# aleju/gan-reverser

Hardware: AMD Instinct MI355X
Metric: images/sec G+R fwd/bwd (higher is better)
Workload: dtype f32 via f16x3 (2-term fp16 split of power-of-two-scaled operands, 3 MFMA products, fp32 accumulate); 1 GPU; 32x32 grayscale, noise=32, batch=256/GPU: G fwd + R fwd/bwd + Adam; global_batch=256, per_gpu_batch=256, parallelism=dp1, bn=per-rank batch statistics

## Files before the change

gan-reverser_amd/csrc/elem.hip:

```cpp
#include "kernels.h"
#include "colorspace.h"
#include <type_traits>

namespace gr {

__device__ __forceinline__ double block_reduce_sum(double v, double* sh) {
#pragma unroll
  for (int off = 32; off > 0; off >>= 1) v += __shfl_down(v, off, 64);
  const int lane = threadIdx.x & 63, wave = threadIdx.x >> 6, nw = (blockDim.x + 63) >> 6;
  __syncthreads();
  if (lane == 0) sh[wave] = v;
  __syncthreads();
  double r = 0;
  if (threadIdx.x == 0) for (int w = 0; w < nw; ++w) r += sh[w];
  return r;
}

__device__ __forceinline__ unsigned udivp(unsigned x, unsigned d) { return (d & (d - 1)) == 0 ? x >> (__ffs(d) - 1) : x / d; }
__device__ __forceinline__ float post_slope(const PostArgs& a) { return a.act == ACT_PRELU ? *a.slope_dev : a.slope; }
template <int CB>
__device__ __forceinline__ void post_specialize(PostArgs& f) {
  if (CB == 1) { f.act = ACT_ELU; f.has_bn = 1; f.m1.kind = MASK_ELEM; f.pool = 0; f.m2.kind = MASK_NONE; }
  if (CB == 2) { f.act = ACT_ELU; f.has_bn = 1; f.m1.kind = MASK_NONE; f.pool = POOL_MAX; f.m2.kind = MASK_ELEM; }
  if (CB == 3) { f.act = ACT_ELU; f.has_bn = 1; f.m1.kind = MASK_SPATIAL; f.pool = POOL_MAX; f.m2.kind = MASK_NONE; }
// ... 1032 lines not shown
  PostBwdArgs a = a0;
  a.nt = 0;
  const PostArgs& f = a.f;
  const double pre = (double)f.B * f.C * f.H * f.W, post = f.pool ? pre / 4 : pre;
  const bool vec = (f.pool ? (f.W % 8 == 0 && f.H % 2 == 0) : (f.W % 4 == 0)) && f.H * f.W >= 64 && pre < 4.0e9;
  if (vec) {
    long blocks = ((long)(pre / 4) + 255) / 256;
    if (blocks > 8192) blocks = 8192;
    KtScope kt("post_backward_frozen_vec_kernel", 0.0, 4.0 * (2.0 * pre + post), s);
    with_combo(post_combo(f), [&](auto cb) { hipLaunchKernelGGL(post_backward_frozen_vec_kernel<decltype(cb)::value>, dim3((unsigned)blocks), dim3(256), 0, s, a); });
  } else {
    long blocks = ((long)pre + 255) / 256;
    if (blocks > 8192) blocks = 8192;
    if (blocks < 1) blocks = 1;
    KtScope kt("post_backward_frozen_kernel", 0.0, 4.0 * (2.0 * pre + post), s);
    hipLaunchKernelGGL(post_backward_frozen_kernel, dim3((unsigned)blocks), dim3(256), 0, s, a);
  }
}

__global__ __launch_bounds__(256) void channel_absmax_kernel(const float* __restrict__ t, int B, long HW, long sB, long sC, unsigned* __restrict__ chmax) {
  const int c = blockIdx.x;
  const long n = (long)B * HW;
  float m = 0.f;
  for (long j = (long)blockIdx.y * 256 + threadIdx.x; j < n; j += (long)gridDim.y * 256) {
    const long b = j / HW, i = j - b * HW;
    m = fmaxf(m, fabsf(t[b * sB + (long)c * sC + i]));
  }
#pragma unroll
  for (int off = 32; off > 0; off >>= 1) m = fmaxf(m, __shfl_down(m, off, 64));
  if ((threadIdx.x & 63) == 0 && m > 0.f) atomicMax(chmax + c, __float_as_uint(m));
}
__device__ __forceinline__ void spread_enter(float mx, float mn, unsigned* word, int side) {
  __shared__ float tmx[256], tmn[256];
  tmx[threadIdx.x] = mx; tmn[threadIdx.x] = mn;
  __syncthreads();
  if (threadIdx.x == 0) {
    for (int i = 1; i < 256; ++i) { mx = fmaxf(mx, tmx[i]); mn = fminf(mn, tmn[i]); }
    if (mx > 0.f && mn < mx) {
      const unsigned bits = (unsigned)min(ilogbf(mx) - ilogbf(mn) + 1, 0xffff);
      const unsigned w = *word;
      unsigned a = w & 0xffffu, b = w >> 16;
      if (side == 0) a = max(a, bits); else b = max(b, bits);
      *word = a | b << 16;
    }
  }
}
__global__ __launch_bounds__(256) void spread_verdict_kernel(unsigned* chmax, int C, unsigned* word, int side) {
  float mx = 0.f, mn = INFINITY;
  for (int c = threadIdx.x; c < C; c += 256) {
    const float v = __uint_as_float(chmax[c]); chmax[c] = 0u;
    mx = fmaxf(mx, v); if (v > 0.f) mn = fminf(mn, v);
  }
  spread_enter(mx, mn, word, side);
}
__global__ __launch_bounds__(256) void pair_spread_kernel(const float* __restrict__ a, const float* __restrict__ b, int C, unsigned* word) {
  float mx = 0.f, mn = INFINITY;
  for (int c = threadIdx.x; c < C; c += 256) {
    const float v = fmaxf(fabsf(a[c]), b ? fabsf(b[c]) : 0.f);
    mx = fmaxf(mx, v); if (v > 0.f) mn = fminf(mn, v);
  }
  spread_enter(mx, mn, word, 0);
}
void launch_channel_absmax(const float* t, int B, int C, long HW, long sB, long sC, unsigned* chmax, hipStream_t s) {
  const long n = (long)B * HW;
  int splits = (int)((n + 4095) / 4096);
  if (splits < 1) splits = 1;
  if ((long)splits * C > 8192) splits = (int)(8192 / C > 0 ? 8192 / C : 1);
  KtScope kt("range_guard_scan", 0.0, 4.0 * (double)n * C, s);
  hipLaunchKernelGGL(channel_absmax_kernel, dim3(C, splits), dim3(256), 0, s, t, B, HW, sB, sC, chmax);
}
void launch_spread_verdict(unsigned* chmax, int C, unsigned* word, int side, hipStream_t s) {
  hipLaunchKernelGGL(spread_verdict_kernel, dim3(1), dim3(256), 0, s, chmax, C, word, side);
}
void launch_pair_spread(const float* a, const float* b, int C, unsigned* sides, hipStream_t s) {
  hipLaunchKernelGGL(pair_spread_kernel, dim3(1), dim3(256), 0, s, a, b, C, sides);
}

__global__ __launch_bounds__(1024) void mse_kernel(const float* __restrict__ x, const float* __restrict__ t, long n, double inv_n,
                                                   float norm, double* loss, float* grad) {
  __shared__ double sh[16];
  double s = 0;
  for (long i = threadIdx.x; i < n; i += blockDim.x) {
    const float z = x[i] - t[i];
    s += (double)(z * z);
    if (grad) grad[i] = norm * z;
  }
  s = block_reduce_sum(s, sh);
  if (threadIdx.x == 0 && loss) *loss = s * inv_n;
}
void launch_mse(const float* x, const float* t, long n, long n_global, double* loss_dev, float* grad, hipStream_t s) {
  hipLaunchKernelGGL(mse_kernel, dim3(1), dim3(1024), 0, s, x, t, n, 1.0 / (double)n_global, (float)(2.0 / (double)n_global), loss_dev, grad);
}

__global__ __launch_bounds__(256) void mse_rows_kernel(const float* __restrict__ x, const float* __restrict__ t, long n, double inv_n, float norm,
                                                       float* __restrict__ loss_rows, float* __restrict__ grad) {
  __shared__ double sh[8];
  const long base = (long)blockIdx.x * n;
  double s = 0;
  for (long j = threadIdx.x; j < n; j += blockDim.x) {
    const float z = x[base + j] - t[base + j];
    s += (double)z * (double)z;
    if (grad) grad[base + j] = norm * z;
  }
  s = block_reduce_sum(s, sh);
  if (threadIdx.x == 0) loss_rows[blockIdx.x] = (float)(s * inv_n);
}
void launch_mse_rows(const float* x, const float* t, long rows, long n, float* loss_rows, float* grad, hipStream_t s) {
  KtScope kt("mse_rows_kernel", 3.0 * (double)rows * n, 4.0 * (double)rows * n * (grad ? 3.0 : 2.0), s);
  hipLaunchKernelGGL(mse_rows_kernel, dim3((unsigned)rows), dim3(256), 0, s, x, t, n, 1.0 / (double)n, (float)(2.0 / (double)n), loss_rows, grad);
}

#define HEAD_KEEP8(a_, i_) asm volatile("" :: "v"((a_)[(i_)]), "v"((a_)[(i_) + 1]), "v"((a_)[(i_) + 2]), "v"((a_)[(i_) + 3]), "v"((a_)[(i_) + 4]), "v"((a_)[(i_) + 5]), "v"((a_)[(i_) + 6]), "v"((a_)[(i_) + 7]))
#define HEAD_KEEP16(a_, i_) asm volatile("" :: "v"((a_)[(i_)]), "v"((a_)[(i_) + 1]), "v"((a_)[(i_) + 2]), "v"((a_)[(i_) + 3]), "v"((a_)[(i_) + 4]), "v"((a_)[(i_) + 5]), "v"((a_)[(i_) + 6]), "v"((a_)[(i_) + 7]), \
                                              "v"((a_)[(i_) + 8]), "v"((a_)[(i_) + 9]), "v"((a_)[(i_) + 10]), "v"((a_)[(i_) + 11]), "v"((a_)[(i_) + 12]), "v"((a_)[(i_) + 13]), "v"((a_)[(i_) + 14]), "v"((a_)[(i_) + 15]))
__device__ __forceinline__ unsigned head_mask_word(const MaskRef& m, long e) { return m.bits[e >> 5]; }
__device__ __forceinline__ float head_mask_of(const MaskRef& m, unsigned w, long e) { const float k = ((w >> (e & 31)) & 1u) ? m.scale : 0.f; return m.kind == MASK_ELEM ? k : 1.f; }
struct HeadArgs {
  int B, C1, nd, rows_per_wg;
  const float* y1; float* out1;
  float* mean; float* invstd; float* run_mean; float* run_var; const float* gamma; const float* beta;
  MaskRef m1; int act1; float slope1; int act2;
  const float* W2; const float* b2; float* y2; float* out2;
  const float* target; double inv_n; float norm; double* loss; double* loss_part;
  float* gout; float* gy2; float* dy1;
  float* gW2; float* gb2; float* ggamma; float* gbeta; float* gb1;
  unsigned* amax_dy;
  unsigned* bar; unsigned bar_base;
  unsigned* fault; int spin_limit;
};
constexpr int HEAD_FW = 8, HEAD_RG = 32, HEAD_RMAX = 16;
__device__ __forceinline__ bool head_grid_barrier(unsigned* ctr, unsigned target, unsigned* fault, int spin_limit) {
  __builtin_amdgcn_fence(__ATOMIC_RELEASE, "agent");
  __syncthreads();
  __shared__ int ok_;
  if (threadIdx.x == 0) {
    __hip_atomic_fetch_add(ctr, 1u, __ATOMIC_RELEASE, __HIP_MEMORY_SCOPE_AGENT);
    int ok = 0;
    for (int spin = 0; spin < spin_limit; ++spin) {
      if ((int)(__hip_atomic_load(ctr, __ATOMIC_ACQUIRE, __HIP_MEMORY_SCOPE_AGENT) - target) >= 0) { ok = 1; break; }
      __builtin_amdgcn_s_sleep(4);
    }
    if (!ok) __hip_atomic_fetch_or(fault, 1u, __ATOMIC_RELEASE, __HIP_MEMORY_SCOPE_AGENT);
    ok_ = ok;
  }
  __syncthreads();
  __builtin_amdgcn_fence(__ATOMIC_ACQUIRE, "agent");
  return ok_ != 0;
}
template <int RT>
__global__ __launch_bounds__(256) __attribute__((amdgpu_waves_per_eu(1, 1))) void head_fwd_bwd_kernel(HeadArgs a) {
  extern __shared__ __attribute__((aligned(16))) unsigned char head_smem[];
  __shared__ double sh_s[HEAD_RG][HEAD_FW], sh_q[HEAD_RG][HEAD_FW];
  __shared__ float sh_mean[HEAD_FW], sh_inv[HEAD_FW], sh_c0[HEAD_FW], sh_c1[HEAD_FW];
  __shared__ double sh_loss8[8];
  const int tid = threadIdx.x, lane = tid & 63, wave = tid >> 6, wg = blockIdx.x, NW = gridDim.x;
  const int B = a.B, C1 = a.C1, nd = a.nd;
  const double n = (double)B;
  bool alive = true;
  const int f0 = wg * HEAD_FW, ff = tid & (HEAD_FW - 1), rg = tid >> 3, f = f0 + ff;
  {
    double s = 0, q = 0;
    for (int b0 = rg; b0 < B; b0 += 8 * HEAD_RG) {
      float v8[8];
#pragma unroll
      for (int u = 0; u < 8; ++u) v8[u] = a.y1[(long)min(b0 + u * HEAD_RG, B - 1) * C1 + f];
      HEAD_KEEP8(v8, 0);
#pragma unroll
      for (int u = 0; u < 8; ++u) { const double v = b0 + u * HEAD_RG < B ? v8[u] : 0.f; s += v; q += v * v; }
    }
    sh_s[rg][ff] = s; sh_q[rg][ff] = q;
    __syncthreads();
    if (tid < HEAD_FW) {
      double ss = 0, qq = 0;
#pragma unroll 8
      for (int k = 0; k < HEAD_RG; ++k) { ss += sh_s[k][tid]; qq += sh_q[k][tid]; }
      const double m = ss / n;
      double vs = qq - ss * m;
      if (vs < 0) vs = 0;
      const float mf = (float)m, is = (float)(1.0 / sqrt(vs / n + 1e-5));
      const int c = f0 + tid;
      a.mean[c] = mf; a.invstd[c] = is;
      if (a.run_mean) {
        a.run_mean[c] = (float)(0.1 * m + 0.9 * (double)a.run_mean[c]);
        a.run_var[c] = (float)(0.1 * (vs / (n - 1)) + 0.9 * (double)a.run_var[c]);
      }
      sh_mean[tid] = mf; sh_inv[tid] = is;
    }
    __syncthreads();
    const float mean = sh_mean[ff], invstd = sh_inv[ff], gm = a.gamma[f], bt = a.beta[f];
    for (int b0 = rg; b0 < B; b0 += 8 * HEAD_RG) {
      float v8[8]; unsigned m8[8];
#pragma unroll
      for (int u = 0; u < 8; ++u) { const long e = (long)min(b0 + u * HEAD_RG, B - 1) * C1 + f; v8[u] = a.y1[e]; m8[u] = head_mask_word(a.m1, e); }
      HEAD_KEEP8(v8, 0); HEAD_KEEP8(m8, 0);
#pragma unroll
      for (int u = 0; u < 8; ++u) {
        const int b = b0 + u * HEAD_RG;
        const long e = (long)min(b, B - 1) * C1 + f;
        const float z = ((v8[u] - mean) * invstd) * gm + bt;
        const float o = act_fwd(z, a.act1, a.slope1) * head_mask_of(a.m1, m8[u], e);
        if (b < B) a.out1[(long)b * C1 + f] = o;
      }
    }
  }
  alive = head_grid_barrier(a.bar, a.bar_base + (unsigned)NW, a.fault, a.spin_limit) && alive;
  const int r0 = wg * RT, nrows = max(0, min(RT, B - r0));
  float* xs = reinterpret_cast<float*>(head_smem);
  float* gy2_s = xs + (size_t)(RT * C1 > B * HEAD_FW ? RT * C1 : B * HEAD_FW);
  float* red = gy2_s + (size_t)RT * nd;
  float* b2_s = red;
  double lacc = 0;
  {
    const int NJ = C1 >> 6;
    const long last1 = (long)B * C1 - 1, last2 = (long)B * nd - 1;
    float xr[2 * RT];
#pragma unroll
    for (int k = 0; k < 2 * RT; ++k) { const long i = (long)r0 * C1 + tid + 256 * k; xr[k] = a.out1[i < last1 ? i : last1]; }
    float w8[8][8];
#pragma unroll
    for (int u = 0; u < 8; ++u)
#pragma unroll
      for (int j = 0; j < 8; ++j) w8[u][j] = a.W2[(long)min(wave + 4 * u, nd - 1) * C1 + lane + 64 * (j < NJ ? j : 0)];
    const float b2r = a.b2[min(tid, nd - 1)];
    float tg[(RT * 128 + 255) / 256];
#pragma unroll
    for (int k = 0; k < (RT * 128 + 255) / 256; ++k) { const long e2 = (long)r0 * nd + tid + 256 * k; tg[k] = a.target[e2 < last2 ? e2 : last2]; }
    float yv[2][RT]; unsigned mk[2][RT];
#pragma unroll
    for (int h2 = 0; h2 < 2; ++h2)
#pragma unroll
      for (int r = 0; r < RT; ++r) { const long e = (long)min(r0 + r, B - 1) * C1 + min(tid + 256 * h2, C1 - 1); yv[h2][r] = a.y1[e]; mk[h2][r] = head_mask_word(a.m1, e); }
    float bnp[2][4];
#pragma unroll
    for (int h2 = 0; h2 < 2; ++h2) { const int fx = min(tid + 256 * h2, C1 - 1); bnp[h2][0] = a.mean[fx]; bnp[h2][1] = a.invstd[fx]; bnp[h2][2] = a.gamma[fx]; bnp[h2][3] = a.beta[fx]; }
#pragma unroll
    for (int k = 0; k < 2 * RT; k += 4) asm volatile("" :: "v"(xr[k]), "v"(xr[k + 1]), "v"(xr[k + 2]), "v"(xr[k + 3]));
#pragma unroll
    for (int u = 0; u < 8; ++u) HEAD_KEEP8(w8[u], 0);
    asm volatile("" :: "v"(b2r), "v"(tg[0]), "v"(bnp[0][0]), "v"(bnp[0][1]), "v"(bnp[0][2]), "v"(bnp[0][3]), "v"(bnp[1][0]), "v"(bnp[1][1]), "v"(bnp[1][2]), "v"(bnp[1][3]));
#pragma unroll
    for (int h2 = 0; h2 < 2; ++h2)
#pragma unroll
      for (int r = 0; r < RT; r += 4) asm volatile("" :: "v"(yv[h2][r]), "v"(yv[h2][r + 1]), "v"(yv[h2][r + 2]), "v"(yv[h2][r + 3]), "v"(mk[h2][r]), "v"(mk[h2][r + 1]), "v"(mk[h2][r + 2]), "v"(mk[h2][r + 3]));
#pragma unroll
    for (int k = 0; k < 2 * RT; ++k) { const int i = tid + 256 * k; if (i < RT * C1) xs[i] = (long)r0 * C1 + i <= last1 ? xr[k] : 0.f; }
    if (tid < nd) b2_s[tid] = b2r;
    __syncthreads();
    for (int ob = wave; ob < nd; ob += 32) {
      float wn[8][8];
      const bool more = ob + 32 < nd;
      if (more) {
#pragma unroll
        for (int u = 0; u < 8; ++u)
#pragma unroll
          for (int j = 0; j < 8; ++j) wn[u][j] = a.W2[(long)min(ob + 32 + 4 * u, nd - 1) * C1 + lane + 64 * (j < NJ ? j : 0)];
      }
#pragma unroll
      for (int u = 0; u < 8; ++u) {
        const int o = ob + 4 * u;
        const float bias2 = b2_s[min(o, nd - 1)];
#pragma unroll
        for (int r = 0; r < RT; ++r) {
          float pr = 0.f;
#pragma unroll
          for (int j = 0; j < 8; ++j) pr = fmaf((o < nd && j < NJ) ? w8[u][j] : 0.f, xs[r * C1 + lane + 64 * (j < NJ ? j : 0)], pr);
          const float v = wave_sum(pr);
          if (lane == 63 && o < nd) gy2_s[r * nd + o] = v + bias2;
        }
      }
      if (more) {
#pragma unroll
        for (int u = 0; u < 8; ++u) HEAD_KEEP8(wn[u], 0);
#pragma unroll
        for (int u = 0; u < 8; ++u)
#pragma unroll
          for (int j = 0; j < 8; ++j) w8[u][j] = wn[u][j];
      }
    }
    float wc[2][32];
#pragma unroll
    for (int h2 = 0; h2 < 2; ++h2)
#pragma unroll
      for (int u = 0; u < 32; ++u) wc[h2][u] = a.W2[(long)min(u, nd - 1) * C1 + min(tid + 256 * h2, C1 - 1)];
    __syncthreads();
#pragma unroll
    for (int k = 0; k < (RT * 128 + 255) / 256; ++k) {
      const int i = tid + 256 * k;
      if (i < nrows * nd) {
        const long e2 = (long)r0 * nd + i;
        const float y = gy2_s[i];
        const float out = act_fwd(y, a.act2, 0.f);
        const float zd = out - tg[k];
        lacc += (double)(zd * zd);
        const float g = a.norm * zd;
        const float g2 = act_bwd(g, y, out, a.act2, 0.f);
        a.y2[e2] = y;
        if (a.out2 != a.y2) a.out2[e2] = out;
        a.gout[e2] = g;
        a.gy2[e2] = g2;
        gy2_s[i] = g2;
      } else if (i < RT * nd) gy2_s[i] = 0.f;
    }
    lacc = block_reduce_sum(lacc, sh_loss8);
    __syncthreads();
    if (tid == 0) a.loss_part[wg] = lacc;
    float acc[2][RT];
#pragma unroll
    for (int h2 = 0; h2 < 2; ++h2)
#pragma unroll
      for (int r = 0; r < RT; ++r) acc[h2][r] = 0.f;
    for (int o0 = 0; o0 < nd; o0 += 32) {
      float wcn[2][32];
      const bool more = o0 + 32 < nd;
      if (more) {
#pragma unroll
        for (int h2 = 0; h2 < 2; ++h2)
#pragma unroll
          for (int u = 0; u < 32; ++u) wcn[h2][u] = a.W2[(long)min(o0 + 32 + u, nd - 1) * C1 + min(tid + 256 * h2, C1 - 1)];
      } else {
#pragma unroll
        for (int h2 = 0; h2 < 2; ++h2) { HEAD_KEEP16(wc[h2], 0); HEAD_KEEP16(wc[h2], 16); }
      }
#pragma unroll
      for (int u = 0; u < 32; ++u) {
        const int oo = min(o0 + u, nd - 1);
        const bool on = o0 + u < nd;
#pragma unroll
        for (int r = 0; r < RT; ++r) {
          const float gv = gy2_s[r * nd + oo];
          acc[0][r] = fmaf(gv, on ? wc[0][u] : 0.f, acc[0][r]);
          acc[1][r] = fmaf(gv, on ? wc[1][u] : 0.f, acc[1][r]);
        }
      }
      if (more) {
#pragma unroll
        for (int h2 = 0; h2 < 2; ++h2) { HEAD_KEEP16(wcn[h2], 0); HEAD_KEEP16(wcn[h2], 16); }
#pragma unroll
        for (int h2 = 0; h2 < 2; ++h2)
#pragma unroll
          for (int u = 0; u < 32; ++u) wc[h2][u] = wcn[h2][u];
      }
    }
#pragma unroll
    for (int h2 = 0; h2 < 2; ++h2) {
      const int fx = tid + 256 * h2;
      const float mean = bnp[h2][0], invstd = bnp[h2][1], gm = bnp[h2][2], bt = bnp[h2][3];
#pragma unroll
      for (int r = 0; r < RT; ++r) {
        const float g = acc[h2][r] * head_mask_of(a.m1, mk[h2][r], (long)min(r0 + r, B - 1) * C1 + min(fx, C1 - 1));
        const float z = ((yv[h2][r] - mean) * invstd) * gm + bt;
        const float dz = act_bwd_z(g, z, a.act1, a.slope1);
        if (r < nrows && fx < C1) a.dy1[(long)(r0 + r) * C1 + fx] = dz;
      }
    }
  }
  alive = head_grid_barrier(a.bar, a.bar_base + 2u * (unsigned)NW, a.fault, a.spin_limit) && alive;
  {
    const float mean = sh_mean[ff], invstd = sh_inv[ff], gm = a.gamma[f];
    double s = 0, q = 0;
    for (int b0 = rg; b0 < B; b0 += 8 * HEAD_RG) {
      float d8[8], y8[8];
#pragma unroll
      for (int u = 0; u < 8; ++u) { const long e = (long)min(b0 + u * HEAD_RG, B - 1) * C1 + f; d8[u] = a.dy1[e]; y8[u] = a.y1[e]; }
      HEAD_KEEP8(d8, 0); HEAD_KEEP8(y8, 0);
#pragma unroll
      for (int u = 0; u < 8; ++u) { const float dz = b0 + u * HEAD_RG < B ? d8[u] : 0.f; s += (double)dz; q += (double)(y8[u] - mean) * (double)dz; }
    }
    __syncthreads();
    sh_s[rg][ff] = s; sh_q[rg][ff] = q;
    __syncthreads();
    if (tid < HEAD_FW) {
      double ss = 0, qq = 0;
#pragma unroll 8
      for (int k = 0; k < HEAD_RG; ++k) { ss += sh_s[k][tid]; qq += sh_q[k][tid]; }
      const double isd = (double)sh_inv[tid];
      const int c = f0 + tid;
      a.ggamma[c] += (float)(qq * isd);
      a.gbeta[c] += (float)ss;
      sh_c0[tid] = (float)(ss / n);
      sh_c1[tid] = (float)(qq * isd * isd / n);
    }
    __syncthreads();
    const float c0 = sh_c0[ff], c1 = sh_c1[ff];
    double sb = 0; float dmax = 0.f;
    for (int b0 = rg; b0 < B; b0 += 8 * HEAD_RG) {
      float d8[8], y8[8];
#pragma unroll
      for (int u = 0; u < 8; ++u) { const long e = (long)min(b0 + u * HEAD_RG, B - 1) * C1 + f; d8[u] = a.dy1[e]; y8[u] = a.y1[e]; }
      HEAD_KEEP8(d8, 0); HEAD_KEEP8(y8, 0);
#pragma unroll
      for (int u = 0; u < 8; ++u) {
        const int b = b0 + u * HEAD_RG;
        const float d = ((d8[u] - c0) - (y8[u] - mean) * c1) * invstd * gm;
        if (b < B) { a.dy1[(long)b * C1 + f] = d; dmax = fmaxf(dmax, fabsf(d)); sb += (double)d; }
      }
    }
    if (a.amax_dy) absmax_commit(dmax, a.amax_dy);
    sh_s[rg][ff] = sb;
    for (int i = tid; i < B * HEAD_FW; i += 256) { const int b = i >> 3, c = i & 7; xs[i] = a.out1[(long)b * C1 + f0 + c]; }
    __syncthreads();
    if (tid < HEAD_FW) {
      double t = 0;
#pragma unroll 8
      for (int k = 0; k < HEAD_RG; ++k) t += sh_s[k][tid];
      a.gb1[f0 + tid] += (float)t;
    }
    const int OG = nd <= 32 ? 32 : (nd <= 64 ? 64 : 128), slices = 256 / OG, o = tid & (OG - 1), sl = tid / OG, oc = min(o, nd - 1);
    float acc[HEAD_FW + 1];
#pragma unroll
    for (int c = 0; c <= HEAD_FW; ++c) acc[c] = 0.f;
    for (int b0 = sl; b0 < B; b0 += 16 * slices) {
      float g16[16];
#pragma unroll
      for (int u = 0; u < 16; ++u) g16[u] = a.gy2[(long)min(b0 + u * slices, B - 1) * nd + oc];
      HEAD_KEEP16(g16, 0);
#pragma unroll
      for (int u = 0; u < 16; ++u) g16[u] = b0 + u * slices < B ? g16[u] : 0.f;
#pragma unroll
      for (int u = 0; u < 16; ++u) {
        const int b = min(b0 + u * slices, B - 1);
        const float g = g16[u];
        const float4 x0 = *reinterpret_cast<const float4*>(xs + b * HEAD_FW), x1 = *reinterpret_cast<const float4*>(xs + b * HEAD_FW + 4);
        acc[0] = fmaf(g, x0.x, acc[0]); acc[1] = fmaf(g, x0.y, acc[1]); acc[2] = fmaf(g, x0.z, acc[2]); acc[3] = fmaf(g, x0.w, acc[3]);
        acc[4] = fmaf(g, x1.x, acc[4]); acc[5] = fmaf(g, x1.y, acc[5]); acc[6] = fmaf(g, x1.z, acc[6]); acc[7] = fmaf(g, x1.w, acc[7]);
        acc[8] += g;
      }
    }
#pragma unroll
    for (int c = 0; c <= HEAD_FW; ++c) red[(sl * OG + o) * (HEAD_FW + 1) + c] = acc[c];
    __syncthreads();
    for (int i = tid; i < nd * (HEAD_FW + 1); i += 256) {
      const int oo = i / (HEAD_FW + 1), c = i - oo * (HEAD_FW + 1);
      float t = 0.f;
      for (int k = 0; k < slices; ++k) t += red[(k * OG + oo) * (HEAD_FW + 1) + c];
      if (c < HEAD_FW) a.gW2[(long)oo * C1 + f0 + c] += t;
      else if (wg == 0) a.gb2[oo] += t;
    }
    if (wg == 0 && tid == 0) {
      double t = 0;
      for (int k = 0; k < NW; ++k) t += a.loss_part[k];
      const bool faulted = !alive || __hip_atomic_load(a.fault, __ATOMIC_ACQUIRE, __HIP_MEMORY_SCOPE_AGENT) != 0u;
      *a.loss = faulted ? (double)NAN : t * a.inv_n;
    }
  }
}
size_t head_lds_bytes(int B, int C1, int nd, int rows_per_wg) {
  const size_t xs = (size_t)(rows_per_wg * C1 > B * HEAD_FW ? rows_per_wg * C1 : B * HEAD_FW);
  return sizeof(float) * (xs + (size_t)rows_per_wg * nd + (size_t)256 * (HEAD_FW + 1));
}
bool head_supported(int B, int C1, int nd) {
  if (B < 2 || C1 % 64 != 0 || C1 < 64 || C1 > 512 || nd < 1 || nd > 128) return false;
  const int NW = C1 / HEAD_FW, R = (B + NW - 1) / NW;
  return R <= 4 && nd <= 32 && head_lds_bytes(B, C1, nd, 4) <= 60 * 1024;
}
void launch_head_fwd_bwd(const HeadLaunch& h, hipStream_t s) {
  HeadArgs a{};
  a.B = h.B; a.C1 = h.C1; a.nd = h.nd;
  const int NW = h.C1 / HEAD_FW;
  a.rows_per_wg = (h.B + NW - 1) / NW;
  a.y1 = h.y1; a.out1 = h.out1; a.mean = h.mean; a.invstd = h.invstd; a.run_mean = h.run_mean; a.run_var = h.run_var; a.gamma = h.gamma; a.beta = h.beta;
  a.m1 = h.m1; if (a.m1.kind != MASK_ELEM) { a.m1.kind = MASK_NONE; a.m1.bits = reinterpret_cast<const uint32_t*>(h.y1); a.m1.scale = 1.f; }
  a.act1 = h.act1; a.slope1 = h.slope1; a.act2 = h.act2;
  a.W2 = h.W2; a.b2 = h.b2; a.y2 = h.y2; a.out2 = h.out2;
  a.target = h.target; a.inv_n = 1.0 / (double)h.n_global; a.norm = (float)(2.0 / (double)h.n_global); a.loss = h.loss; a.loss_part = h.loss_part;
  a.gout = h.gout; a.gy2 = h.gy2; a.dy1 = h.dy1;
  a.gW2 = h.gW2; a.gb2 = h.gb2; a.ggamma = h.ggamma; a.gbeta = h.gbeta; a.gb1 = h.gb1;
  a.amax_dy = h.amax_dy; a.bar = h.bar; a.bar_base = h.bar_base; a.fault = h.fault; a.spin_limit = h.spin_limit > 0 ? h.spin_limit : (1 << 22);
  const size_t lds = head_lds_bytes(h.B, h.C1, h.nd, 4);
  static bool attr = false;
  if (!attr) { (void)hipFuncSetAttribute(reinterpret_cast<const void*>(&head_fwd_bwd_kernel<4>), hipFuncAttributeMaxDynamicSharedMemorySize, 64 * 1024); attr = true; }
  KtScope kt("head_fwd_bwd_kernel", 2.0 * 3.0 * h.B * (double)h.C1 * h.nd, 4.0 * (6.0 * h.B * h.C1 + 3.0 * (double)h.nd * h.C1), s);
  hipLaunchKernelGGL(head_fwd_bwd_kernel<4>, dim3(NW), dim3(256), lds, s, a);
}

__global__ __launch_bounds__(1024) void bce_kernel(const float* __restrict__ x, const float* __restrict__ t, long n, double* loss, float* grad) {
  __shared__ double sh[16];
  const double EPS = 1e-12, norm = 1.0 / (double)n;
  double s = 0;
  for (long i = threadIdx.x; i < n; i += blockDim.x) {
    const double xv = (double)x[i], tv = (double)t[i];
    s -= log(xv + EPS) * tv + log(1. - xv + EPS) * (1. - tv);
    if (grad) grad[i] = (float)(-norm * (tv - xv) / ((1. - xv + EPS) * (xv + EPS)));
  }
  s = block_reduce_sum(s, sh);
  if (threadIdx.x == 0 && loss) *loss = s * norm;
}
void launch_bce(const float* x, const float* t, long n, double* loss_dev, float* grad, hipStream_t s) {
  hipLaunchKernelGGL(bce_kernel, dim3(1), dim3(1024), 0, s, x, t, n, loss_dev, grad);
}

__global__ void add_inplace_kernel(float* __restrict__ y, const float* __restrict__ x, long n) {
  for (long i = blockIdx.x * (long)blockDim.x + threadIdx.x; i < n; i += (long)gridDim.x * blockDim.x) y[i] = y[i] + x[i];
}
void launch_add_inplace(float* y, const float* x, long n, hipStream_t s) {
  if (n <= 0) return;
  const long blocks = (n + 255) / 256;
  hipLaunchKernelGGL(add_inplace_kernel, dim3((unsigned)(blocks < 2048 ? blocks : 2048)), dim3(256), 0, s, y, x, n);
}

template <class Consts>
__device__ __forceinline__ void penalty_clamp_one(const float th, float& gv, const Consts& c) {
  if (c.use_penalty) {
    const float sg = th > 0.f ? 1.f : (th < 0.f ? -1.f : 0.f);
    const float pen = sg * c.l1 + th * c.l2;
    gv = gv + pen;
  }
  if (c.use_clamp) gv = gv < -c.clamp ? -c.clamp : (gv > c.clamp ? c.clamp : gv);
}
__device__ __forceinline__ void adam_one(float& th, float& gv, float& mv, float& vv, const AdamConsts& c) {
  penalty_clamp_one(th, gv, c);
  mv = mv * c.b1 + c.c1 * gv;
  vv = vv * c.b2 + (c.c2 * gv) * gv;
  const float denom = sqrtf(vv) + c.eps;
  th = th + (c.step * mv) / denom;
}
__global__ __launch_bounds__(256) void penalty_clamp_adam_kernel(float* __restrict__ theta, float* __restrict__ g, float* __restrict__ m,
                                                                 float* __restrict__ v, long n, AdamConsts c, const unsigned* __restrict__ skip) {
  if (skip != nullptr && *skip != 0u) return;
  const long n4 = n >> 2;
  for (long i = blockIdx.x * (long)blockDim.x + threadIdx.x; i <= n4; i += (long)gridDim.x * blockDim.x) {
    if (i < n4) {
      float4 th = reinterpret_cast<float4*>(theta)[i], gv = reinterpret_cast<float4*>(g)[i];
      float4 mv = reinterpret_cast<float4*>(m)[i], vv = reinterpret_cast<float4*>(v)[i];
      adam_one(th.x, gv.x, mv.x, vv.x, c); adam_one(th.y, gv.y, mv.y, vv.y, c);
      adam_one(th.z, gv.z, mv.z, vv.z, c); adam_one(th.w, gv.w, mv.w, vv.w, c);
      reinterpret_cast<float4*>(theta)[i] = th; reinterpret_cast<float4*>(g)[i] = gv;
      reinterpret_cast<float4*>(m)[i] = mv; reinterpret_cast<float4*>(v)[i] = vv;
    } else {
      for (long j = n4 << 2; j < n; ++j) {
        float th = theta[j], gv = g[j], mv = m[j], vv = v[j];
        adam_one(th, gv, mv, vv, c);
        theta[j] = th; g[j] = gv; m[j] = mv; v[j] = vv;
      }
    }
  }
}
void launch_penalty_clamp_adam(float* theta, float* g, float* m, float* v, long n, const AdamConsts& c, hipStream_t s, const unsigned* skip) {
  long blocks = ((n >> 2) + 1 + 255) / 256;
  if (blocks > 4096) blocks = 4096;
  if (blocks < 1) blocks = 1;
  KtScope kt("penalty_clamp_adam_kernel", 0.0, 32.0 * (double)n, s);
  hipLaunchKernelGGL(penalty_clamp_adam_kernel, dim3((unsigned)blocks), dim3(256), 0, s, theta, g, m, v, n, c, skip);
}

__global__ __launch_bounds__(256) void adam_rows_kernel(float* __restrict__ z, float* __restrict__ g, float* __restrict__ m, float* __restrict__ v, int rows, int nd,
                                                        AdamConsts c, float zclamp, const float* __restrict__ loss_rows, float* __restrict__ best_loss,
                                                        float* __restrict__ best_z, int update) {
  for (int r = blockIdx.x; r < rows; r += gridDim.x) {
    const bool better = loss_rows[r] < best_loss[r];
    __syncthreads();
    if (better && threadIdx.x == 0) best_loss[r] = loss_rows[r];
    const long base = (long)r * nd;
    for (int j = threadIdx.x; j < nd; j += blockDim.x) {
      float th = z[base + j];
      if (better) best_z[base + j] = th;
      if (update) {
        float gv = g[base + j], mv = m[base + j], vv = v[base + j];
        adam_one(th, gv, mv, vv, c);
        if (zclamp > 0.f) th = th < -zclamp ? -zclamp : (th > zclamp ? zclamp : th);
        z[base + j] = th; m[base + j] = mv; v[base + j] = vv;
      }
    }
  }
}
void launch_adam_rows(float* z, float* g, float* m, float* v, int rows, int nd, const AdamConsts& c, float zclamp, const float* loss_rows, float* best_loss,
                      float* best_z, int update, hipStream_t s) {
  KtScope kt("adam_rows_kernel", 0.0, 4.0 * (double)rows * nd * (update ? 8.0 : 2.0), s);
  hipLaunchKernelGGL(adam_rows_kernel, dim3((unsigned)(rows < 4096 ? rows : 4096)), dim3(256), 0, s, z, g, m, v, rows, nd, c, zclamp, loss_rows, best_loss, best_z, update);
}

template <int M, bool MOM>
__device__ __forceinline__ void optim_one(float& th, float& gv, float& a, float& b, const OptimConsts& c) {
  penalty_clamp_one(th, gv, c);
  if constexpr (M == OPT_SGD) {
    float d = gv;
    if (c.use_wd) d = d + c.wd * th;
    if constexpr (MOM) {
      a = c.first ? d : c.mom * a + c.omd * d;
      d = c.nesterov ? d + c.mom * a : a;
    }
    th = th - c.lr * d;
  } else if constexpr (M == OPT_ADAGRAD) {
    a = a + gv * gv;
    th = th - (c.lr * gv) / (sqrtf(a) + 1e-10f);
  } else if constexpr (M == OPT_ADADELTA) {
    a = c.rho * a + (c.omr * gv) * gv;
    const float sd = sqrtf(a + c.eps);
    const float delta = sqrtf(b + c.eps) / sd * gv;
    th = th - delta;
    b = c.rho * b + (c.omr * delta) * delta;
  } else if constexpr (M == OPT_ADAMAX) {
    a = c.b1 * a + c.c1 * gv;
    const float x = c.b2 * b, y = fabsf(gv) + c.eps;
    b = x != x ? x : (y != y ? y : (x > y ? x : y));
    th = th - (c.lr * a) / b;
  } else {
    static_assert(M == OPT_RMSPROP, "unknown method");
    a = c.rho * a + (c.omr * gv) * gv;
    th = th - (c.lr * gv) / (sqrtf(a) + c.eps);
  }
}
// ... 299 lines not shown
```

Baseline: 132,800 images/sec.

## Keep head y1/out1 tile on-chip across phases and prefetch bwd loads early

```diff
diff --git a/gan-reverser_amd/csrc/elem.hip b/gan-reverser_amd/csrc/elem.hip
--- a/gan-reverser_amd/csrc/elem.hip
+++ b/gan-reverser_amd/csrc/elem.hip
@@ -1208,22 +1208,26 @@
   extern __shared__ __attribute__((aligned(16))) unsigned char head_smem[];
   __shared__ double sh_s[HEAD_RG][HEAD_FW], sh_q[HEAD_RG][HEAD_FW];
   __shared__ float sh_mean[HEAD_FW], sh_inv[HEAD_FW], sh_c0[HEAD_FW], sh_c1[HEAD_FW];
-  __shared__ double sh_loss8[8];
+  __shared__ double sh_loss8[8], sh_lpart[64];
   const int tid = threadIdx.x, lane = tid & 63, wave = tid >> 6, wg = blockIdx.x, NW = gridDim.x;
   const int B = a.B, C1 = a.C1, nd = a.nd;
   const double n = (double)B;
   bool alive = true;
   const int f0 = wg * HEAD_FW, ff = tid & (HEAD_FW - 1), rg = tid >> 3, f = f0 + ff;
+  float* const o1_s = reinterpret_cast<float*>(head_smem);
+  float y8[8];
+  const float gm1 = a.gamma[f];
   {
+    unsigned m8[8];
+#pragma unroll
+    for (int u = 0; u < 8; ++u) { const long e = (long)min(rg + u * HEAD_RG, B - 1) * C1 + f; y8[u] = a.y1[e]; m8[u] = head_mask_word(a.m1, e); }
+    const float bt = a.beta[f];
+    const float rm_old = (a.run_mean ? a.run_mean : a.gamma)[f], rv_old = (a.run_mean ? a.run_var : a.gamma)[f];
+    HEAD_KEEP8(y8, 0); HEAD_KEEP8(m8, 0);
+    asm volatile("" :: "v"(gm1), "v"(bt), "v"(rm_old), "v"(rv_old));
     double s = 0, q = 0;
-    for (int b0 = rg; b0 < B; b0 += 8 * HEAD_RG) {
-      float v8[8];
-#pragma unroll
-      for (int u = 0; u < 8; ++u) v8[u] = a.y1[(long)min(b0 + u * HEAD_RG, B - 1) * C1 + f];
-      HEAD_KEEP8(v8, 0);
-#pragma unroll
-      for (int u = 0; u < 8; ++u) { const double v = b0 + u * HEAD_RG < B ? v8[u] : 0.f; s += v; q += v * v; }
-    }
+#pragma unroll
+    for (int u = 0; u < 8; ++u) { const double v = rg + u * HEAD_RG < B ? y8[u] : 0.f; s += v; q += v * v; }
     sh_s[rg][ff] = s; sh_q[rg][ff] = q;
     __syncthreads();
     if (tid < HEAD_FW) {
@@ -1237,32 +1241,26 @@
       const int c = f0 + tid;
       a.mean[c] = mf; a.invstd[c] = is;
       if (a.run_mean) {
-        a.run_mean[c] = (float)(0.1 * m + 0.9 * (double)a.run_mean[c]);
-        a.run_var[c] = (float)(0.1 * (vs / (n - 1)) + 0.9 * (double)a.run_var[c]);
+        a.run_mean[c] = (float)(0.1 * m + 0.9 * (double)rm_old);
+        a.run_var[c] = (float)(0.1 * (vs / (n - 1)) + 0.9 * (double)rv_old);
       }
       sh_mean[tid] = mf; sh_inv[tid] = is;
     }
     __syncthreads();
-    const float mean = sh_mean[ff], invstd = sh_inv[ff], gm = a.gamma[f], bt = a.beta[f];
-    for (int b0 = rg; b0 < B; b0 += 8 * HEAD_RG) {
-      float v8[8]; unsigned m8[8];
-#pragma unroll
-      for (int u = 0; u < 8; ++u) { const long e = (long)min(b0 + u * HEAD_RG, B - 1) * C1 + f; v8[u] = a.y1[e]; m8[u] = head_mask_word(a.m1, e); }
-      HEAD_KEEP8(v8, 0); HEAD_KEEP8(m8, 0);
-#pragma unroll
-      for (int u = 0; u < 8; ++u) {
-        const int b = b0 + u * HEAD_RG;
-        const long e = (long)min(b, B - 1) * C1 + f;
-        const float z = ((v8[u] - mean) * invstd) * gm + bt;
-        const float o = act_fwd(z, a.act1, a.slope1) * head_mask_of(a.m1, m8[u], e);
-        if (b < B) a.out1[(long)b * C1 + f] = o;
-      }
+    const float mean = sh_mean[ff], invstd = sh_inv[ff];
+#pragma unroll
+    for (int u = 0; u < 8; ++u) {
+      const int b = rg + u * HEAD_RG;
+      const long e = (long)min(b, B - 1) * C1 + f;
+      const float z = ((y8[u] - mean) * invstd) * gm1 + bt;
+      const float o = act_fwd(z, a.act1, a.slope1) * head_mask_of(a.m1, m8[u], e);
+      if (b < B) { a.out1[(long)b * C1 + f] = o; o1_s[b * HEAD_FW + ff] = o; }
     }
   }
   alive = head_grid_barrier(a.bar, a.bar_base + (unsigned)NW, a.fault, a.spin_limit) && alive;
   const int r0 = wg * RT, nrows = max(0, min(RT, B - r0));
-  float* xs = reinterpret_cast<float*>(head_smem);
-  float* gy2_s = xs + (size_t)(RT * C1 > B * HEAD_FW ? RT * C1 : B * HEAD_FW);
+  float* xs = o1_s + (size_t)B * HEAD_FW;
+  float* gy2_s = xs + (size_t)RT * C1;
   float* red = gy2_s + (size_t)RT * nd;
   float* b2_s = red;
   double lacc = 0;
@@ -1412,16 +1410,26 @@
   }
   alive = head_grid_barrier(a.bar, a.bar_base + 2u * (unsigned)NW, a.fault, a.spin_limit) && alive;
   {
-    const float mean = sh_mean[ff], invstd = sh_inv[ff], gm = a.gamma[f];
+    const float mean = sh_mean[ff], invstd = sh_inv[ff];
+    const int OG = nd <= 32 ? 32 : (nd <= 64 ? 64 : 128), slices = 256 / OG, o = tid & (OG - 1), sl = tid / OG, oc = min(o, nd - 1);
+    const int NGW = nd * (HEAD_FW + 1);
+    auto grad_old = [&](int i) -> float* { i = min(i, NGW - 1); const int oo = i / (HEAD_FW + 1), c = i - oo * (HEAD_FW + 1); return c < HEAD_FW ? a.gW2 + (long)oo * C1 + f0 + c : a.gb2 + oo; };
+    float d8[8], gp[2][16];
+#pragma unroll
+    for (int u = 0; u < 8; ++u) d8[u] = a.dy1[(long)min(rg + u * HEAD_RG, B - 1) * C1 + f];
+#pragma unroll
+    for (int it = 0; it < 2; ++it)
+#pragma unroll
+      for (int u = 0; u < 16; ++u) gp[it][u] = a.gy2[(long)min(sl + (16 * it + u) * slices, B - 1) * nd + oc];
+    const float gg_old = a.ggamma[f], gbt_old = a.gbeta[f], gb1_old = a.gb1[f];
+    const float gw_old0 = *grad_old(tid), gw_old1 = *grad_old(tid + 256);
+    const double lpart = a.loss_part[min(tid, NW - 1)];
+    HEAD_KEEP8(d8, 0); HEAD_KEEP16(gp[0], 0); HEAD_KEEP16(gp[1], 0);
+    asm volatile("" :: "v"(gg_old), "v"(gbt_old), "v"(gb1_old), "v"(gw_old0), "v"(gw_old1), "v"(lpart));
+    if (tid < 64) sh_lpart[tid] = lpart;
     double s = 0, q = 0;
-    for (int b0 = rg; b0 < B; b0 += 8 * HEAD_RG) {
-      float d8[8], y8[8];
-#pragma unroll
-      for (int u = 0; u < 8; ++u) { const long e = (long)min(b0 + u * HEAD_RG, B - 1) * C1 + f; d8[u] = a.dy1[e]; y8[u] = a.y1[e]; }
-      HEAD_KEEP8(d8, 0); HEAD_KEEP8(y8, 0);
-#pragma unroll
-      for (int u = 0; u < 8; ++u) { const float dz = b0 + u * HEAD_RG < B ? d8[u] : 0.f; s += (double)dz; q += (double)(y8[u] - mean) * (double)dz; }
-    }
+#pragma unroll
+    for (int u = 0; u < 8; ++u) { const float dz = rg + u * HEAD_RG < B ? d8[u] : 0.f; s += (double)dz; q += (double)(y8[u] - mean) * (double)dz; }
     __syncthreads();
     sh_s[rg][ff] = s; sh_q[rg][ff] = q;
     __syncthreads();
@@ -1431,78 +1439,76 @@
       for (int k = 0; k < HEAD_RG; ++k) { ss += sh_s[k][tid]; qq += sh_q[k][tid]; }
       const double isd = (double)sh_inv[tid];
       const int c = f0 + tid;
-      a.ggamma[c] += (float)(qq * isd);
-      a.gbeta[c] += (float)ss;
+      a.ggamma[c] = gg_old + (float)(qq * isd);
+      a.gbeta[c] = gbt_old + (float)ss;
       sh_c0[tid] = (float)(ss / n);
       sh_c1[tid] = (float)(qq * isd * isd / n);
     }
     __syncthreads();
     const float c0 = sh_c0[ff], c1 = sh_c1[ff];
     double sb = 0; float dmax = 0.f;
-    for (int b0 = rg; b0 < B; b0 += 8 * HEAD_RG) {
-      float d8[8], y8[8];
-#pragma unroll
-      for (int u = 0; u < 8; ++u) { const long e = (long)min(b0 + u * HEAD_RG, B - 1) * C1 + f; d8[u] = a.dy1[e]; y8[u] = a.y1[e]; }
-      HEAD_KEEP8(d8, 0); HEAD_KEEP8(y8, 0);
-#pragma unroll
-      for (int u = 0; u < 8; ++u) {
-        const int b = b0 + u * HEAD_RG;
-        const float d = ((d8[u] - c0) - (y8[u] - mean) * c1) * invstd * gm;
-        if (b < B) { a.dy1[(long)b * C1 + f] = d; dmax = fmaxf(dmax, fabsf(d)); sb += (double)d; }
-      }
+#pragma unroll
+    for (int u = 0; u < 8; ++u) {
+      const int b = rg + u * HEAD_RG;
+      const float d = ((d8[u] - c0) - (y8[u] - mean) * c1) * invstd * gm1;
+      if (b < B) { a.dy1[(long)b * C1 + f] = d; dmax = fmaxf(dmax, fabsf(d)); sb += (double)d; }
     }
     if (a.amax_dy) absmax_commit(dmax, a.amax_dy);
     sh_s[rg][ff] = sb;
-    for (int i = tid; i < B * HEAD_FW; i += 256) { const int b = i >> 3, c = i & 7; xs[i] = a.out1[(long)b * C1 + f0 + c]; }
     __syncthreads();
     if (tid < HEAD_FW) {
       double t = 0;
 #pragma unroll 8
       for (int k = 0; k < HEAD_RG; ++k) t += sh_s[k][tid];
-      a.gb1[f0 + tid] += (float)t;
-    }
-    const int OG = nd <= 32 ? 32 : (nd <= 64 ? 64 : 128), slices = 256 / OG, o = tid & (OG - 1), sl = tid / OG, oc = min(o, nd - 1);
+      a.gb1[f0 + tid] = gb1_old + (float)t;
+    }
     float acc[HEAD_FW + 1];
 #pragma unroll
     for (int c = 0; c <= HEAD_FW; ++c) acc[c] = 0.f;
-    for (int b0 = sl; b0 < B; b0 += 16 * slices) {
+    auto rows16 = [&](int b0, const float (&gl)[16]) {
       float g16[16];
 #pragma unroll
-      for (int u = 0; u < 16; ++u) g16[u] = a.gy2[(long)min(b0 + u * slices, B - 1) * nd + oc];
-      HEAD_KEEP16(g16, 0);
-#pragma unroll
-      for (int u = 0; u < 16; ++u) g16[u] = b0 + u * slices < B ? g16[u] : 0.f;
+      for (int u = 0; u < 16; ++u) g16[u] = b0 + u * slices < B ? gl[u] : 0.f;
 #pragma unroll
       for (int u = 0; u < 16; ++u) {
         const int b = min(b0 + u * slices, B - 1);
         const float g = g16[u];
-        const float4 x0 = *reinterpret_cast<const float4*>(xs + b * HEAD_FW), x1 = *reinterpret_cast<const float4*>(xs + b * HEAD_FW + 4);
+        const float4 x0 = *reinterpret_cast<const float4*>(o1_s + b * HEAD_FW), x1 = *reinterpret_cast<const float4*>(o1_s + b * HEAD_FW + 4);
         acc[0] = fmaf(g, x0.x, acc[0]); acc[1] = fmaf(g, x0.y, acc[1]); acc[2] = fmaf(g, x0.z, acc[2]); acc[3] = fmaf(g, x0.w, acc[3]);
         acc[4] = fmaf(g, x1.x, acc[4]); acc[5] = fmaf(g, x1.y, acc[5]); acc[6] = fmaf(g, x1.z, acc[6]); acc[7] = fmaf(g, x1.w, acc[7]);
         acc[8] += g;
       }
+    };
+    if (sl < B) rows16(sl, gp[0]);
+    if (sl + 16 * slices < B) rows16(sl + 16 * slices, gp[1]);
+    for (int b0 = sl + 32 * slices; b0 < B; b0 += 16 * slices) {
+      float g16[16];
+#pragma unroll
+      for (int u = 0; u < 16; ++u) g16[u] = a.gy2[(long)min(b0 + u * slices, B - 1) * nd + oc];
+      HEAD_KEEP16(g16, 0);
+      rows16(b0, g16);
     }
 #pragma unroll
     for (int c = 0; c <= HEAD_FW; ++c) red[(sl * OG + o) * (HEAD_FW + 1) + c] = acc[c];
     __syncthreads();
-    for (int i = tid; i < nd * (HEAD_FW + 1); i += 256) {
+    for (int i = tid; i < NGW; i += 256) {
       const int oo = i / (HEAD_FW + 1), c = i - oo * (HEAD_FW + 1);
       float t = 0.f;
       for (int k = 0; k < slices; ++k) t += red[(k * OG + oo) * (HEAD_FW + 1) + c];
-      if (c < HEAD_FW) a.gW2[(long)oo * C1 + f0 + c] += t;
-      else if (wg == 0) a.gb2[oo] += t;
+      float* const p = grad_old(i);
+      const float old = i == tid ? gw_old0 : (i == tid + 256 ? gw_old1 : *p);
+      if (c < HEAD_FW || wg == 0) *p = old + t;
     }
     if (wg == 0 && tid == 0) {
       double t = 0;
-      for (int k = 0; k < NW; ++k) t += a.loss_part[k];
+      for (int k = 0; k < NW; ++k) t += sh_lpart[k];
       const bool faulted = !alive || __hip_atomic_load(a.fault, __ATOMIC_ACQUIRE, __HIP_MEMORY_SCOPE_AGENT) != 0u;
       *a.loss = faulted ? (double)NAN : t * a.inv_n;
     }
   }
 }
 size_t head_lds_bytes(int B, int C1, int nd, int rows_per_wg) {
-  const size_t xs = (size_t)(rows_per_wg * C1 > B * HEAD_FW ? rows_per_wg * C1 : B * HEAD_FW);
-  return sizeof(float) * (xs + (size_t)rows_per_wg * nd + (size_t)256 * (HEAD_FW + 1));
+  return sizeof(float) * ((size_t)B * HEAD_FW + (size_t)rows_per_wg * C1 + (size_t)rows_per_wg * nd + (size_t)256 * (HEAD_FW + 1));
 }
 bool head_supported(int B, int C1, int nd) {
   if (B < 2 || C1 % 64 != 0 || C1 < 64 || C1 > 512 || nd < 1 || nd > 128) return false;
```

Result: no change. 133,300 images/sec (median of 6 runs) (+0.4%).
